# flybirdxx/ComfyUI-SDMatte

Measured on AMD Instinct MI355X. Metric: alpha mattes/sec at 1024x1024, higher is better.
Workload: dtype f16x3

## Files before the change

comfyui-sdmatte_amd/csrc/sdm_engine.cpp:

```cpp
#include "sdm_common.h"
#include "k_conv.h"
#include "k_gemm.h"
#include "k_norm.h"
#include "k_attn.h"
#include "k_misc.h"
#include "k_trimap.h"
#include "k_cclabel.h"
#include "k_foreground.h"
#include "k_guided.h"
#include "k_temporal.h"
#include "k_motion.h"
#include "k_defocus.h"
#include "k_plate.h"
#include "k_harmonize.h"
#include "k_key.h"
#include "k_metrics.h"
#include "k_roi.h"
#include "k_canvas.h"
#include "k_boxes.h"
#include "k_tiles.h"
#include "k_distance.h"
#include "../../include/sdmatte.h"

#include <algorithm>
// ... 65 lines not shown
  {"gemm_p3", 1, 1, "transformer-block Linear layers on the plane-fed GEMM (k_gemm.h): pre-split operand planes from LayerNorm / GroupNorm / attention / GEGLU, LDS-DMA only (the W3 weight copies are built when a model is built)"},
  {"gemm_p3_tile", 0, 0, "row tile of the plane-fed GEMM: 0 by shape, 256 / 128 / 64 forced"},
  {"gemm_p3_attn", 1, 1, "d=64 attention cores write the operand planes of to_out themselves (0: fp32 result + one conversion pass)"},
  {"gemm_p3_persist", 1, 1, "plane-fed GEMM: persistent blocks that prefetch the next tile's first chunk underneath the epilogue (0: one block per tile, n > 1: a grid of n blocks - tests)"},
  {"gemm_p3_ablate", 0, 0, "bench only: 1 no MFMAs, 2 no DMAs behind the prologue, 4 no epilogue (sdm_bench_gemm_p3)"},
  {"conv_up_phase", 1, 1, "up-sampling 3x3 convs (Upsample2D) as four 2x2-tap phase convs on the plane-fed GEMM (k_gemm.h, UP): 0 off (the 3x3 kernels on the up-sampled image), 1 the launches with at least two 256-row tiles per CU (up_phase_wins: measured), 2 every eligible launch (tests).  0 / non-0 is read when a model is built: the phase matrices are a derived weight layout"},
  {"conv_epi", 4, 4, "F8 kernels' epilogue: 4 register-direct stores + residual as accumulator init, 3 residual init only, 0 LDS-staged"},
  {"conv_xtile", 1, 1, "F8 3x3: cross-tile prefetch by the producer waves"},
  {"conv_f8_tpb", 0, 0, "F8: tiles per block (0 = by queue depth)"},
  {"conv_dma", 1, 1, "3x3 stride-1 256x128 tile: weights by LDS-DMA"},
  {"conv_dma_all", 0, 0, "keep a stage-ordered weight copy for every wide 3x3 layer, not only the split-precision ones (read when a model is built)"},
  {"conv_pc", -1, -1, "producer / consumer form of the split-precision DMA kernel: -1 by channel count, 0 off, 1 on"},
  {"conv_pc_min_cin", 256, 256, "conv_pc = -1: smallest Cin that takes the producer / consumer form"},
  {"conv_db", 0, 0, "512x128 double-buffered tile where the queue is deep"},
  {"trimap_skip", 1, 1, "VAE encoder, trimap images: output tiles inside a constant region of the trimap are not multiplied (k_misc.h cmask_*; exact). 0 = every tile"},
  {"conv_band_rows", 0, 0, "tile rows per XCD band of the convs that leave constant tiles out (0 = by image height)"},
  {"trimap_skip_min_rows", 512, 512, "smallest output height at which constant tiles are left out (measured at 1024^2: the 1024- and 512-row levels gain 3.7 + 1.6 ms, the 256-row level loses 0.7: too few of its 32 x 128-pixel tiles lie inside one region)"},
  {"conv_splitk", -1, -1, "split-K of the register-staged conv / GEMM kernels: -1 by shape (few tiles, long K), 0 off, n >= 2 forced where the shape allows"},
  {"force_cfg0", 0, 0, "always the 256x128 tile for 3x3 stride 1 (tests: fused GroupNorm at tiny sizes)"},
  {"no_gn_fuse", 0, 0, "never fuse the GroupNorm apply into the consuming conv"},
  {"split_lds_pad", 0, 0, "extra dynamic LDS of the register-staged split kernels (forces one block per CU)"},
  {"attn_f8", 1, 1, "Q.K^T residual terms of the d=64 split-precision attention on fp8 MFMAs"},
  {"attn_dense", 0, 0, "walk every key tile of the trimap-biased self-attention"},
  {"attn_pv_split", 0, 0, "residual terms of P.V too (fully split attention; tests)"},
  {"attn_nw", 0, 0, "waves per d=64 attention block: 0 by launch size, 4, 8"},
  {"attn_pipe", 1, 1, "8-wave split-precision d=64 attention: two-tile software pipeline"},
  {"attn_pipe4", 1, 1, "the same pipeline for the 4-wave launches (two K / three V^T buffers)"},
  {"attn_pp", 1, 1, "split-precision d=64 attention with fp32 output as a ping-pong of the block's wave halves (attn_d64_pp_kernel, 256 query rows per block): 0 off, 1 on, 2 on without the static priority of the younger half, 3 on with per-segment priority flips"},
  {"attn_pp_min_blocks", 128, 128, "attn_pp: launches with fewer 256-row blocks than this keep the 4-wave pipelines (0 in tests: the ping-pong kernel at any size)"},
  {"attn_ksplit", 0, 0, "key split of the d=64 split-precision attention: 0 by launch size (blocks that do not fill the chip's block slots a whole number of times), 1 off, 2 / 4 forced, 3 forced on the ping-pong kernel (ignored elsewhere: those launches run unsplit)"},
// ... 473 lines not shown
#endif
};

struct sdm_ctx {
  sdm_config cfg;
  int device = 0;
  const unsigned char* dbg_cmask = nullptr;
  void* stream = nullptr;
  bool own_stream = false;
  std::string err;
  std::vector<ConvL> convs;
  std::vector<NormL> norms;
  std::unordered_map<std::string, Slot> slots;
  std::vector<std::string> slot_order;
  unsigned char* warena = nullptr;
  size_t warena_bytes = 0, canon_bytes = 0;
  std::vector<float> hostblob;
  int64_t n_loaded = 0, n_ignored = 0;
  std::vector<std::string> missing;
  bool finalized = false;
  void* stage = nullptr;
  size_t stage_bytes = 0;
  struct LoadSlot {
    void* host = nullptr; void* dev = nullptr; size_t cap = 0; bool busy = false;
#ifndef SDM_EMU
    hipEvent_t done = nullptr;
#endif
  };
  static const int kLoadSlots = 3;
  LoadSlot load_ring[kLoadSlots];
// ... 267 lines not shown
  const int nl = c.unet_layers_per_block + 1;
  for (int i = 0; i < 4; ++i) {
    const int prev_out = output_channel;
    output_channel = uc[3 - i];
    const int input_channel = uc[3 - std::min(i + 1, 3)];
    for (int j = 0; j < nl; ++j) {
      const int res_skip = (j == nl - 1) ? input_channel : output_channel;
      const int resnet_in = (j == 0) ? prev_out : output_channel;
      e->u_up_res[i].push_back(B.resnet("unet.up_blocks." + S(i) + ".resnets." + S(j), resnet_in + res_skip, output_channel, te));
      if (i > 0) e->u_up_tf[i].push_back(B.transformer("unet.up_blocks." + S(i) + ".attentions." + S(j), output_channel, c.unet_heads[3 - i], ctx));
    }
    if (i < 3) e->u_up_us.push_back(B.conv_named("unet.up_blocks." + S(i) + ".upsamplers.0.conv", 9, output_channel, output_channel, true, 0, 0, 1));
  }
  e->u_norm_out = B.norm_named("unet.conv_norm_out", uc[0]);
  e->u_conv_out = B.conv_named("unet.conv_out", 9, uc[0], c.unet_out_channels);
  e->canon_bytes = B.woff;
  e->warena_bytes = B.woff + B.doff;
}

static const size_t kAsideOff = (size_t)1 << 62;

static void arena_diverged(sdm_ctx* e, const char* fmt, size_t i, size_t a, size_t b) {
  if (e->adiverged) return;
  char buf[256];
  snprintf(buf, sizeof(buf), fmt, i, a, b);
  e->adiverged = true; e->adiv_msg = buf;
}

static T talloc_aside(sdm_ctx* e, T t) {
  void* p = nullptr;
// ... 1076 lines not shown
  TRY(conv_simple(e, e->enc_conv_in, xin, &h, e->cfg.vae_channels[0], e->cfg.stream_f32, 1, 0, 0, nullptr, 1.0f, true));
  if (cm) tfree_raw(e, xin.cm_off, xin.cm_bytes);
  for (int i = 0; i < 4; ++i) {
    for (auto& r : e->enc_res[i]) { TRY(resblock(e, r, h, nullptr, eps, &t)); tfree(e, h); h = t; }
    if (i < 3) { TRY(conv_simple(e, e->enc_down[i], h, &t, e->cfg.vae_channels[i], e->cfg.stream_f32, 2, 1, 0, nullptr, 1.0f, true)); tfree(e, h); h = t; }
  }
  TRY(resblock(e, e->enc_mid0, h, nullptr, eps, &t)); tfree(e, h); h = t;
  TRY(vae_attention(e, e->enc_attn, h, &t)); tfree(e, h); h = t;
  TRY(resblock(e, e->enc_mid1, h, nullptr, eps, &t)); tfree(e, h); h = t;
  *moments = talloc(e, h.N, h.H, h.W, 16, e->act_f32);
  { ConvArgs a; a.out = moments; TRY(gn_conv(e, e->norms[e->enc_norm_out], e->convs[e->enc_conv_out], h, nullptr, 1, eps, a)); }
  tfree(e, h);
  return 0;
}

static int vae_decode(sdm_ctx* e, const T& z, T* dec) {
  const float eps = e->cfg.vae_eps;
  T h, t;
  TRY(conv_simple(e, e->dec_conv_in, z, &h, e->cfg.vae_channels[3], e->cfg.stream_f32, 1, 0, 0, nullptr, 1.0f, true));
  TRY(resblock(e, e->dec_mid0, h, nullptr, eps, &t)); tfree(e, h); h = t;
  TRY(vae_attention(e, e->dec_attn, h, &t)); tfree(e, h); h = t;
  TRY(resblock(e, e->dec_mid1, h, nullptr, eps, &t)); tfree(e, h); h = t;
  for (int i = 0; i < 4; ++i) {
    for (auto& r : e->dec_res[i]) { TRY(resblock(e, r, h, nullptr, eps, &t)); tfree(e, h); h = t; }
    if (i < 3) { TRY(conv_simple(e, e->dec_up[i], h, &t, e->cfg.vae_channels[3 - i], e->cfg.stream_f32, 1, 0, 1, nullptr, 1.0f, true)); tfree(e, h); h = t; }
  }
  *dec = talloc(e, h.N, h.H, h.W, 4, 1);
  { ConvArgs a; a.out = dec; TRY(gn_conv(e, e->norms[e->dec_norm_out], e->convs[e->dec_conv_out], h, nullptr, 1, eps, a)); }
  tfree(e, h);
  return 0;
}

static bool level_patch_tokens(sdm_ctx* e, int k, int H, int W, bool option_on) {
  if (!option_on || !sdm_patch_tokens_ok(H, W)) return false;
  const int pf = unet_attn_plane_fmt(e);
  bool ok = true;
  if (k < 3) for (auto& t : e->u_down_tf[k]) ok = ok && transformer_p3(e, t, pf);
  if (k == 3) ok = ok && transformer_p3(e, e->u_midtf, pf);
  if (k < 3) for (auto& t : e->u_up_tf[3 - k]) ok = ok && transformer_p3(e, t, pf);
  return ok;
}

static int unet_forward(sdm_ctx* e, const T& uin, bool masked, float* const* bias_lvl, int* const* tiles_lvl, const bool* patch_lvl, T* out) {
// ... 73 lines not shown
  T uin = talloc(e, B, lh, lw, 16, e->act_f32);
  if (!e->dry) SDM_CHECK_DEV(e, dev_memset(uin.p, 0, uin.bytes, e->stream));
  for (int half = 0; half < 2; ++half) {
    T mv = moments; mv.N = B;
    if (!e->dry) mv.p = (unsigned char*)moments.p + (size_t)half * B * lh * lw * 16 * fmt_bytes(moments.f32);
    ConvArgs a; a.in0 = &mv; a.out = &uin; a.out_ch_off = half * 4; a.cout_valid = 4; a.out_scale = c.vae_scaling_factor;
    TRY(op_conv(e, e->convs[e->quant], a));
  }
  tfree(e, moments);
  T lat;
  TRY(unet_forward(e, uin, use_mask, bias_lvl, tiles_lvl, patch_lvl, &lat));
  tfree(e, uin);
  for (int k = 3; k >= 0; --k) { tfree(e, tilebuf[k]); tfree(e, biasbuf[k]); }
  T z;
  TRY(conv_simple(e, e->post_quant, lat, &z, 16, e->act_f32)); tfree(e, lat);
  T dec;
  TRY(vae_decode(e, z, &dec)); tfree(e, z);
  *alpha = talloc(e, B, SH, SW, 1, 1);
  if (!e->dry)
    SDM_LAUNCH(alpha_out_kernel, dim3((unsigned)(((long)B * SH * SW + 255) / 256)), dim3(256), 0, e->stream, (const float*)dec.p, (float*)alpha->p,
               (long)B * SH * SW);
  tfree(e, dec);
  return 0;
}

static int trimap_check(sdm_ctx* e, int B, int H, int W, int erode_px, int dilate_px) {
  if (B <= 0 || H <= 0 || W <= 0) SDM_FAIL(e, SDM_ERR_INVALID, "trimap from mask: bad mask size %dx%dx%d", B, H, W);
  if (erode_px < 0 || erode_px > SDM_TRIMAP_MAX_RADIUS || dilate_px < 0 || dilate_px > SDM_TRIMAP_MAX_RADIUS)
    SDM_FAIL(e, SDM_ERR_INVALID, "trimap from mask: erode_px = %d, dilate_px = %d outside 0 .. %d", erode_px, dilate_px, SDM_TRIMAP_MAX_RADIUS);
  if ((double)B * H * sdm_cdiv(W, SDM_TRIMAP_ROWS_W) >= 2147483647.0) SDM_FAIL(e, SDM_ERR_INVALID, "trimap from mask: %dx%dx%d is too large", B, H, W);
  return 0;
}

static int trimap_cols_rows(int B, int H, int W, int R) {
  int rows = 128;
  while (rows > 32 && ((long)B * sdm_cdiv(H, rows) * sdm_cdiv(W, SDM_TRIMAP_COLS_W) < 512 || trimap_cols_smem(rows, R) > 48 * 1024)) rows /= 2;
  return rows;
// ... 333 lines not shown
  (void)hipEventCreate(&e->ev0); (void)hipEventCreate(&e->ev1);
  (void)hipEventCreateWithFlags(&e->ev_in, hipEventDisableTiming); (void)hipEventCreateWithFlags(&e->ev_out, hipEventDisableTiming);
#endif
  void* p = nullptr;
  if (dev_malloc(&p, e->warena_bytes) != 0) { g_create_err = "cannot allocate weight arena"; sdm_destroy(e); return SDM_ERR_NOMEM; }
  e->warena = (unsigned char*)p;
  dev_memset(e->warena, 0, e->warena_bytes, e->stream);
  for (auto& L : e->convs) {
    L.w = (half_t*)(e->warena + L.w_off); L.b = (float*)(e->warena + L.b_off);
    if (L.split) L.w_lo = (half_t*)(e->warena + L.wlo_off);
    if (L.wdma_bytes) L.w_dma = (half_t*)(e->warena + e->canon_bytes + L.wdma_off);
    if (L.w3_bytes) L.w3 = e->warena + e->canon_bytes + L.w3_off;
    if (L.wup_bytes) L.wup = e->warena + e->canon_bytes + L.wup_off;
  }
  for (auto& n : e->norms) { n.g = (float*)(e->warena + n.g_off); n.b = (float*)(e->warena + n.b_off); }
  for (auto& t : e->tembs) {
    void* q = nullptr;
    if (dev_malloc(&q, (size_t)kMinVariantRows * t.cout_pad * 4) != 0) { g_create_err = "cannot allocate temb tables"; sdm_destroy(e); return SDM_ERR_NOMEM; }
    t.table = (float*)q;
    dev_memset(q, 0, (size_t)kMinVariantRows * t.cout_pad * 4, e->stream);
  }
  e->variant_cap = kMinVariantRows;
  dev_sync(e->stream);
  *out = e;
  return SDM_OK;
}

void sdm_destroy(sdm_ctx* e) {
  if (e) dev_use(e->device);
  if (!e) return;
// ... 267 lines not shown
                 (const half_t*)L->w, (const half_t*)L->w_lo, L->wup, L->Cin_pad, L->Cout_pad, ldexpf(1.0f, -L->w_exp), ldexpf(1.0f, L->up_exp));
    if (!L->w_dma) continue;
    const size_t total = (size_t)L->Cin_pad * L->ntaps * L->Cout_pad;
    if (L->f8)
      SDM_LAUNCH(derive_conv_weight_f8_kernel, dim3((unsigned)std::min<size_t>((total / 4 + 255) / 256, 65535)), dim3(256), 0, e->stream,
                 (const half_t*)L->w, (const half_t*)L->w_lo, (unsigned char*)L->w_dma, L->Cin_pad, L->Cout_pad, L->ntaps, ldexpf(1.0f, -L->w_exp),
                 ldexpf(1.0f, L->f8_exp));
    else
      SDM_LAUNCH(derive_conv_weight_dma_kernel, dim3((unsigned)std::min<size_t>((total * (L->split ? 2 : 1) + 255) / 256, 65535)), dim3(256), 0, e->stream,
                 (const half_t*)L->w, (const half_t*)L->w_lo, L->w_dma, L->Cin_pad, L->Cout_pad, L->split ? 2 : 1);
  }
  SDM_CHECK_DEV(e, dev_sync(e->stream));
  return 0;
}

static void load_ring_release(sdm_ctx* e) {
#ifndef SDM_EMU
  for (auto& sl : e->load_ring) {
    if (sl.busy) { (void)hipEventSynchronize(sl.done); sl.busy = false; }
    if (sl.host) (void)hipHostFree(sl.host);
    if (sl.dev) dev_free(sl.dev);
    if (sl.done) (void)hipEventDestroy(sl.done);
    sl.host = sl.dev = nullptr; sl.cap = 0; sl.done = nullptr;
  }
#else
  (void)e;
#endif
}

int sdm_finalize_weights(sdm_ctx* e) {
  if (e) dev_use(e->device);
  if (!e) return SDM_ERR_INVALID;
  SDM_CHECK_DEV(e, dev_sync(e->stream));
  load_ring_release(e);
  { int rc = fold_cross_kv(e); if (rc) return rc; }
  {
    std::vector<ConvL*> all;
    for (auto& L : e->convs) all.push_back(&L);
    int rc = derive_layers(e, all);
    if (rc) return rc;
  }
  e->missing.clear();
  for (auto& k : e->slot_order) if (!e->slots[k].loaded) e->missing.push_back(k);
  e->variants.clear();
  e->finalized = true;
  return SDM_OK;
}

int sdm_weight_stats(sdm_ctx* e, int64_t* n_loaded, int64_t* n_missing, int64_t* n_ignored) {
  if (!e) return SDM_ERR_INVALID;
  if (n_loaded) *n_loaded = e->n_loaded;
  if (n_missing) *n_missing = (int64_t)e->missing.size();
  if (n_ignored) *n_ignored = e->n_ignored;
  return SDM_OK;
// ... 1335 lines not shown
```

comfyui-sdmatte_amd/csrc/sdm_hooks.h:

```cpp
#pragma once

struct DevBuf {
  void* p = nullptr;
  DevBuf() = default;
  DevBuf(DevBuf&& o) noexcept : p(o.p) { o.p = nullptr; }
  ~DevBuf() { if (p) dev_free(p); }
  int alloc(size_t n) { return dev_malloc(&p, n); }
  int alloc0(size_t n, void* stream) { const int rc = alloc(n); return rc ? rc : dev_memset(p, 0, n, stream); }
};

struct RestoreInt { int& s; int v; ~RestoreInt() { s = v; } };

struct TempLayer {
  enum { kDma = 1, kW3 = 2, kUp = 4 };
  sdm_ctx* e;
  ConvL L;
  DevBuf w, w_lo, b, w_dma, w3, wup;
  explicit TempLayer(sdm_ctx* c) : e(c) {}
  ~TempLayer() { dev_sync(e->stream); }
  int init(const char* name, int ntaps, int I, int O, int geglu, int split, int layouts, const float* wsrc, const float* bias) {
    L = make_layer(name, ntaps, I, O, geglu, split);
    layer_choose_layouts(L, layouts & kDma, layouts & kDma, layouts & kW3, layouts & kUp);
    SDM_CHECK_DEV(e, w.alloc0(L.w_bytes(), e->stream));
    SDM_CHECK_DEV(e, b.alloc0(L.b_bytes(), e->stream));
// ... 236 lines not shown
  TRY(tl.init("op_up", 9, C, O, 0, 1, TempLayer::kDma | TempLayer::kUp, w, bias));
  return run_two_pass(e, [&]() -> int {
    T tin = view(x, N, H, W, C, 1), to = view(out, N, 2 * H, 2 * W, O, 1);
    to.want_stats = true;
    ConvArgs a; a.in0 = &tin; a.out = &to; a.up = 1;
    TRY(op_conv(e, tl.L, a));
    if (!e->dry) {
      SDM_CHECK_DEV(e, dev_memcpy_d2d(stats, to.stats, (size_t)N * to.srows * O * 2 * 4, e->stream));
      *srows = to.srows;
    }
    if (to.sbytes) { tfree_raw(e, to.soff, to.sbytes); to.sbytes = 0; }
    return 0;
  });
}

int sdm_debug_set_input_cmask(sdm_ctx* e, const unsigned char* mask) {
  if (!e) return SDM_ERR_INVALID;
  e->dbg_cmask = mask;
  return SDM_OK;
}

int sdm_op_conv(sdm_ctx* e, const void* in0, const void* in1, int C0, int C1, int in_f32, int N, int Hin, int Win, int up, int stride,
                int pad_mode, int ntaps, const float* w, const float* bias, int O, void* out, int out_f32, const void* res, int res_f32,
                int geglu, float out_scale, int tile_cfg) {
  return sdm_op_conv_ex(e, in0, in1, C0, C1, in_f32, N, Hin, Win, up, stride, pad_mode, ntaps, w, bias, O, out, out_f32, res, res_f32, geglu,
                        out_scale, tile_cfg, 0, nullptr, nullptr, 0.0f, 32, 0);
}


int sdm_debug_run_layer(sdm_ctx* e, const char* layer_name, const float* x, int N, int H, int W, float* out, int Cout) {
// ... 477 lines not shown
```

comfyui-sdmatte_amd/engine.py:

```python
import ctypes as C
import os

import numpy as np
import torch

from .config import SDMatteConfig

_HERE = os.path.dirname(os.path.abspath(__file__))
LIB_PATH = os.path.join(_HERE, "csrc", "libsdmatte_hip.so")

SDM_PTR_HOST, SDM_PTR_DEVICE = 0, 1
SDM_F32, SDM_F16, SDM_BF16 = 0, 1, 2
_DT = {torch.float32: SDM_F32, torch.float16: SDM_F16, torch.bfloat16: SDM_BF16}


class SdmConfig(C.Structure):
    _fields_ = [
        ("vae_channels", C.c_int32 * 4), ("vae_layers_per_block", C.c_int32),
        ("unet_channels", C.c_int32 * 4), ("unet_heads", C.c_int32 * 4), ("unet_layers_per_block", C.c_int32),
        ("cross_attention_dim", C.c_int32), ("unet_in_channels", C.c_int32), ("unet_out_channels", C.c_int32),
        ("bbox_embeddings_input_dim", C.c_int32), ("groups", C.c_int32),
        ("vae_eps", C.c_float), ("unet_res_eps", C.c_float), ("unet_tf_gn_eps", C.c_float), ("unet_ln_eps", C.c_float),
        ("vae_scaling_factor", C.c_float), ("attn_mask_value", C.c_float),
        ("stream_f32", C.c_int32), ("point_embeddings_input_dim", C.c_int32), ("precise_mask", C.c_int32), ("reserved", C.c_int32 * 5),
# ... 36 lines not shown
    c.unet_tf_gn_eps, c.unet_ln_eps = cfg.unet_tf_gn_eps, cfg.unet_ln_eps
    c.vae_scaling_factor, c.attn_mask_value = cfg.vae_scaling_factor, cfg.attn_mask_value
    c.stream_f32 = 1 if stream_f32 else 0
    c.point_embeddings_input_dim = cfg.point_embeddings_input_dim
    c.precise_mask = precise_mask_of(precision)
    return c


EXPORTS = [
    "sdm_default_config", "sdm_create", "sdm_destroy", "sdm_last_error", "sdm_load_tensor", "sdm_finalize_weights",
    "sdm_weight_stats", "sdm_missing_key", "sdm_weight_blob_bytes", "sdm_export_weight_blob", "sdm_import_weight_blob",
    "sdm_host_blob_bytes", "sdm_export_host_blob", "sdm_import_host_blob", "sdm_forward", "sdm_forward_ex", "sdm_forward_rect", "sdm_apply_matte", "sdm_apply_matte_node",
    "sdm_make_trimap", "sdm_clean_mask", "sdm_apply_matte_mask", "sdm_subject_roi", "sdm_apply_matte_roi", "sdm_subject_boxes", "sdm_apply_matte_boxes", "sdm_band_tiles", "sdm_apply_matte_tiles", "sdm_estimate_foreground", "sdm_refine_alpha_guided", "sdm_compose_canvas",
    "sdm_distance_field", "sdm_offset_mask", "sdm_outline", "sdm_smooth_alpha_temporal", "sdm_smooth_alpha_motion", "sdm_defocus_background", "sdm_fill_background", "sdm_harmonize", "sdm_screen_colour", "sdm_chroma_key", "sdm_matte_metrics",
    "sdm_synchronize", "sdm_release_memory", "sdm_resident_bytes", "sdm_weight_bytes", "sdm_last_forward_ms", "sdm_profile_enable", "sdm_profile_count", "sdm_profile_get", "sdm_profile_dump",
    "sdm_op_conv", "sdm_op_conv_ex", "sdm_op_conv_stats", "sdm_op_gn_partials", "sdm_op_gn_tables", "sdm_op_conv_up_stats", "sdm_op_gemm_p3", "sdm_debug_run_layer", "sdm_debug_set_input_cmask", "sdm_debug_temb_row", "sdm_conv_num_cfgs", "sdm_bench_conv", "sdm_bench_attn", "sdm_bench_gemm_p3", "sdm_op_groupnorm", "sdm_op_layernorm", "sdm_op_attention", "sdm_op_attention_ex", "sdm_op_attention_split", "sdm_op_attention_split_ex", "sdm_debug_attn_plan", "sdm_op_resize_aa",
    "sdm_op_mask_bias", "sdm_debug_patch_token_map", "sdm_op_groupnorm_p3", "sdm_op_gemm_p3_tokens", "sdm_op_mask_bias_tokens", "sdm_op_active_tiles",
    "sdm_op_cross_patch_planes", "sdm_op_cross_patch_planes_ex", "sdm_op_attention_shared", "sdm_debug_cross_attention", "sdm_op_cross_core",
    "sdm_set_option", "sdm_get_option", "sdm_reset_options", "sdm_option_name", "sdm_option_help", "sdm_kernel_counts", "sdm_kernel_counts_reset",
]


class Bindings:

    def __init__(self, cdll):
        self.dll = cdll
        vp, i32, i64, f32 = C.c_void_p, C.c_int, C.c_int64, C.c_float
        sig = {
            "sdm_default_config": (None, [C.POINTER(SdmConfig)]),
            "sdm_create": (i32, [C.POINTER(vp), i32, C.POINTER(SdmConfig)]),
            "sdm_destroy": (None, [vp]),
# ... 44 lines not shown
            "sdm_profile_enable": (i32, [vp, i32]),
            "sdm_profile_count": (i32, [vp]),
            "sdm_profile_dump": (C.c_char_p, [vp]),
            "sdm_profile_get": (i32, [vp, i32, C.POINTER(C.c_char_p), C.POINTER(f32), C.POINTER(i64), C.POINTER(C.c_double),
                                      C.POINTER(C.c_double)]),
            "sdm_op_conv": (i32, [vp, vp, vp, i32, i32, i32, i32, i32, i32, i32, i32, i32, i32, vp, vp, i32, vp, i32, vp, i32, i32,
                                  f32, i32]),
            "sdm_op_conv_ex": (i32, [vp, vp, vp, i32, i32, i32, i32, i32, i32, i32, i32, i32, i32, vp, vp, i32, vp, i32, vp, i32, i32,
                                     f32, i32, i32, vp, vp, f32, i32, i32]),
            "sdm_op_conv_stats": (i32, [vp, vp, vp, i32, i32, i32, i32, i32, i32, i32, i32, i32, i32, vp, vp, i32, vp, i32, vp, i32, i32,
                                        f32, i32, i32, vp, vp, f32, i32, i32, vp, i32, vp, i32, vp, i32, C.POINTER(i32)]),
            "sdm_op_gn_partials": (i32, [vp, vp, i32, vp, i32, i32, i32, i32, i32, i32, vp, vp, f32, vp, vp]),
            "sdm_op_gn_tables": (i32, [vp, vp, vp, i32, i32, i32, i32, i32, i32, vp, vp, f32, vp, vp]),
            "sdm_op_gemm_p3": (i32, [vp, vp, i32, i32, i32, i32, vp, vp, i32, i32, vp, vp, vp, f32, i32, vp, vp, C.POINTER(i32)]),
            "sdm_op_conv_up_stats": (i32, [vp, vp, i32, i32, i32, i32, vp, vp, i32, vp, vp, C.POINTER(i32)]),
            "sdm_debug_run_layer": (i32, [vp, C.c_char_p, vp, i32, i32, i32, vp, i32]),
            "sdm_debug_set_input_cmask": (i32, [vp, vp]),
            "sdm_debug_temb_row": (i32, [vp, i32, i32, vp, vp, i32]),
            "sdm_conv_num_cfgs": (i32, [i32, i32]),
            "sdm_bench_conv": (f32, [vp] + [i32] * 11),
            "sdm_bench_attn": (f32, [vp] + [i32] * 7),
            "sdm_bench_gemm_p3": (f32, [vp, C.c_long, i32, i32, i32, i32]),
            "sdm_op_groupnorm": (i32, [vp, vp, vp, i32, i32, i32, i32, i32, i32, vp, vp, f32, i32, vp]),
            "sdm_op_layernorm": (i32, [vp, vp, i32, C.c_long, i32, vp, vp, f32, vp]),
            "sdm_op_attention": (i32, [vp, vp, i32, vp, i32, vp, i32, vp, i32, i32, i32, i32, i32, vp, i32]),
            "sdm_op_attention_ex": (i32, [vp, vp, i32, vp, i32, vp, i32, i32, i32, i32, i32, i32, i32, vp, i32]),
            "sdm_op_attention_split": (i32, [vp, vp, vp, vp, vp, i32, i32, i32, i32, vp]),
            "sdm_op_attention_split_ex": (i32, [vp, vp, vp, vp, vp, vp, i32, i32, i32, i32, i32, vp, vp]),
            "sdm_debug_attn_plan": (i32, [i32] * 10 + [C.c_char_p, i32, C.POINTER(i32)]),
            "sdm_op_resize_aa": (i32, [vp, vp, i32, i32, i32, vp, i32, i32]),
# ... 1200 lines not shown
        return scale, shift

    def op_conv_up_stats(self, x, w, bias=None):
        N, H, W_, Cin = x.shape
        O = w.shape[0]
        x = x.float().contiguous(); w = w.float().contiguous()
        b = bias.float().contiguous() if bias is not None else None
        out = torch.empty(N, 2 * H, 2 * W_, O, dtype=torch.float32, device=x.device)
        srows_max = 8 * (((H + 2) * (W_ + 2) + 63) // 64) + 4 * ((H + 1) // 2) * ((W_ + 3) // 4)
        stats = torch.zeros(N * srows_max * O * 2, dtype=torch.float32, device=x.device)
        srows = C.c_int(0)
        self._check(self.lib.sdm_op_conv_up_stats(self.h, _ptr(x), N, H, W_, Cin, _ptr(w), _ptr(b), O, _ptr(out), _ptr(stats), C.byref(srows)),
                    "sdm_op_conv_up_stats")
        return out, stats[:N * srows.value * O * 2].view(N, srows.value, O, 2)

    def op_gemm_p3(self, x, w, bias=None, mode=0, res=None, ln=None, lo_cols=-1):
        N, H, W_, K = x.shape
        O = w.shape[0]
        x = x.float().contiguous(); w = w.float().contiguous()
        b = bias.float().contiguous() if bias is not None else None
        r = res.float().contiguous() if res is not None else None
        gam = ln[0].float().contiguous() if ln is not None else None
        bet = ln[1].float().contiguous() if ln is not None else None
        Cst = O // 2 if mode == 1 else O
        if mode == 2:
            out = torch.zeros(2 * N * H * W_ * O, dtype=torch.float16, device=x.device)
        else:
            out = torch.empty(N, H, W_, Cst, dtype=torch.float32, device=x.device)
        srows_max = 2 * ((H * W_ + 63) // 64)
        stats = torch.zeros(N * srows_max * O * 2, dtype=torch.float32, device=x.device) if mode == 4 else None
# ... 176 lines not shown
```

include/sdmatte.h:

```cpp
#ifndef SDMATTE_H_
#define SDMATTE_H_

#include <stddef.h>
#include <stdint.h>

#ifdef __cplusplus
extern "C" {
#endif

typedef struct sdm_ctx sdm_ctx;

enum sdm_status {
  SDM_OK = 0,
  SDM_ERR_INVALID = -1,
  SDM_ERR_HIP = -2,
  SDM_ERR_STATE = -3,
  SDM_ERR_NOMEM = -4,
  SDM_ERR_NODEVICE = -5,
  SDM_ERR_ARENA = -6
};

enum sdm_ptr_kind { SDM_PTR_HOST = 0, SDM_PTR_DEVICE = 1 };
enum sdm_dtype { SDM_F32 = 0, SDM_F16 = 1, SDM_BF16 = 2 };

// ... 231 lines not shown
                   const float* gn_beta, float gn_eps, int gn_groups, int gn_silu);
int sdm_op_conv_stats(sdm_ctx* ctx, const void* in0, const void* in1, int C0, int C1, int in_f32, int N, int Hin, int Win, int up,
                      int stride, int pad_mode, int ntaps, const float* w, const float* bias, int O, void* out, int out_f32,
                      const void* res, int res_f32, int geglu, float out_scale, int tile_cfg, int split, const float* gn_gamma,
                      const float* gn_beta, float gn_eps, int gn_groups, int gn_silu, const float* in_st0, int in_rows0, const float* in_st1,
                      int in_rows1, float* stats, int stats_cap, int* srows);
int sdm_op_gn_partials(sdm_ctx* ctx, const float* st0, int rows0, const float* st1, int rows1, int C0, int C1, int N, int HW, int groups,
                       const float* gamma, const float* beta, float eps, float* scale, float* shift);
int sdm_op_gn_tables(sdm_ctx* ctx, const void* x0, const void* x1, int C0, int C1, int in_f32, int N, int HW, int groups, const float* gamma,
                     const float* beta, float eps, float* scale, float* shift);
float sdm_bench_gemm_p3(sdm_ctx* ctx, long M, int K, int O, int epi_flags, int iters);
int sdm_op_gemm_p3(sdm_ctx* ctx, const float* x, int N, int H, int W, int K, const float* w, const float* bias, int O, int mode, const float* res,
                   const float* ln_gamma, const float* ln_beta, float ln_eps, int lo_cols, void* out, float* stats, int* srows);
int sdm_op_conv_up_stats(sdm_ctx* ctx, const float* x, int N, int H, int W, int C, const float* w, const float* bias, int O, float* out, float* stats,
                         int* srows);
int sdm_debug_set_input_cmask(sdm_ctx* ctx, const unsigned char* mask);
int sdm_debug_run_layer(sdm_ctx* ctx, const char* layer_name, const float* x_nhwc, int N, int H, int W, float* out_nhwc, int Cout);
int sdm_debug_temb_row(sdm_ctx* ctx, int temb_index, int is_trans, const float* coords4, float* out_host, int cout);
float sdm_bench_attn(sdm_ctx* ctx, int B, int heads, int Lq, int Lk, int qt, int ablate, int iters);
float sdm_bench_conv(sdm_ctx* ctx, int N, int H, int W, int Cin, int Cout, int ntaps, int stride, int in_f32, int tile_cfg, int ablate, int iters);
int sdm_op_groupnorm(sdm_ctx* ctx, const void* in0, const void* in1, int C0, int C1, int in_f32, int N, int HW, int groups,
                     const float* gamma, const float* beta, float eps, int silu, void* out_f16);
int sdm_op_layernorm(sdm_ctx* ctx, const void* x, int in_f32, long rows, int C, const float* gamma, const float* beta,
                     float eps, void* out_f16);
int sdm_op_attention(sdm_ctx* ctx, const void* q, int ldq, const void* k, int ldk, const void* v, int ldv, const float* bias,
                     int B, int heads, int Lq, int Lk, int D, void* out, int ldo);
int sdm_op_attention_ex(sdm_ctx* ctx, const void* q, int ldq, const void* k, int ldk, const void* v, int ldv, int B, int heads, int Lq, int Lk, int D, int out_f32,
                        void* out, int ldo);
int sdm_op_attention_split(sdm_ctx* ctx, const float* q, const float* k, const float* v, const float* bias, int B, int heads, int Lq, int Lk, float* out);
int sdm_op_attention_split_ex(sdm_ctx* ctx, const float* q, const float* k, const float* v, const float* bias, const int* tiles, int B, int heads, int Lq,
// ... 23 lines not shown
```

Before: 22.00.

## Fuse VAE decoder tail into one alpha kernel on mean-folded conv_out weights

New measurement: 22.05 (median of 6 runs). About the same (+0.2%).

```diff
diff --git a/comfyui-sdmatte_amd/csrc/k_vae_ends.h b/comfyui-sdmatte_amd/csrc/k_vae_ends.h
--- /dev/null
+++ b/comfyui-sdmatte_amd/csrc/k_vae_ends.h
@@ -0,0 +1,138 @@
+#pragma once
+#include "sdm_common.h"
+
+#define SDM_DA_TH 30
+#define SDM_DA_TW 32
+#define SDM_DA_RH (SDM_DA_TH + 2)
+#define SDM_DA_RW (SDM_DA_TW + 2)
+#define SDM_DA_RWP (SDM_DA_RW + 1)
+#define SDM_DA_U 4
+
+struct DecAlphaParams {
+  const float* x;
+  const float* scale;
+  const float* shift;
+  const float* wt;
+  float* alpha;
+  int N, H, W;
+};
+
+template <int LPP>
+SDM_DEV_INLINE float dec_alpha_group_sum(float v) {
+#ifdef SDM_EMU
+#pragma unroll
+  for (int m = 1; m < LPP; m <<= 1) v += __shfl_xor(v, m);
+#else
+  v = SDM_DPP_ADD(v, 0xB1);
+  v = SDM_DPP_ADD(v, 0x4E);
+  if (LPP >= 8) v = SDM_DPP_ADD(v, 0x141);
+  if (LPP >= 16) v = SDM_DPP_ADD(v, 0x140);
+#endif
+  return v;
+}
+
+SDM_DEV_INLINE float dec_alpha_silu(float x) {
+  const float d = 1.0f + sdm_exp2(fminf(-x * SDM_LOG2E, 126.0f));
+  float r = sdm_rcp(d);
+  r = fmaf(fmaf(-d, r, 1.0f), r, r);
+  return x * r;
+}
+
+template <int C>
+__global__ void __launch_bounds__(256, 2) dec_alpha_kernel(DecAlphaParams p) {
+  constexpr int LPP = C / 8, PPB = 256 / LPP, NPIX = SDM_DA_RH * SDM_DA_RW, STEPS = (NPIX + PPB - 1) / PPB, NB = (STEPS + SDM_DA_U - 1) / SDM_DA_U;
+  static_assert(C == 32 || C == 64 || C == 128, "dec_alpha_kernel: 4, 8 or 16 lanes per pixel");
+  SDM_SHARED float t[9 * SDM_DA_RH * SDM_DA_RWP];
+  const int tid = threadIdx.x, j = tid % LPP, g = tid / LPP;
+  const int n = blockIdx.z, y0 = blockIdx.y * SDM_DA_TH, x0 = blockIdx.x * SDM_DA_TW;
+  const int H = p.H, W = p.W;
+  const int th = min(SDM_DA_TH, H - y0), tw = min(SDM_DA_TW, W - x0);
+  f32x4 w[9][2], sc[2], sh[2];
+#pragma unroll
+  for (int h = 0; h < 2; ++h) {
+#pragma unroll
+    for (int tap = 0; tap < 9; ++tap) w[tap][h] = *(const f32x4*)(p.wt + tap * C + 4 * (j + h * LPP));
+    sc[h] = *(const f32x4*)(p.scale + (size_t)n * C + 4 * (j + h * LPP));
+    sh[h] = *(const f32x4*)(p.shift + (size_t)n * C + 4 * (j + h * LPP));
+  }
+  const float* img = p.x + (size_t)n * H * W * C;
+  auto place = [&](int pix, int& pr, int& pc) -> bool {
+    pr = pix / SDM_DA_RW; pc = pix - pr * SDM_DA_RW;
+    const int gy = y0 - 1 + pr, gx = x0 - 1 + pc;
+    return pix < NPIX && pr < th + 2 && pc < tw + 2 && gy >= 0 && gy < H && gx >= 0 && gx < W;
+  };
+  auto load = [&](f32x4 (&a)[SDM_DA_U][2], int batch) {
+#pragma unroll
+    for (int u = 0; u < SDM_DA_U; ++u) {
+      int pr, pc;
+      (void)place((batch * SDM_DA_U + u) * PPB + g, pr, pc);
+      pr = min(pr, SDM_DA_RH - 1);
+      const int gy = min(max(y0 - 1 + pr, 0), H - 1), gx = min(max(x0 - 1 + pc, 0), W - 1);
+      const f32x4* s = (const f32x4*)(img + ((size_t)gy * W + gx) * C) + j;
+      a[u][0] = s[0]; a[u][1] = s[LPP];
+    }
+  };
+  auto compute = [&](const f32x4 (&a)[SDM_DA_U][2], int batch) {
+#pragma unroll
+    for (int u = 0; u < SDM_DA_U; ++u) {
+      const int pix = (batch * SDM_DA_U + u) * PPB + g;
+      int pr, pc;
+      const bool ok = place(pix, pr, pc);
+      float v[8];
+#pragma unroll
+      for (int h = 0; h < 2; ++h)
+#pragma unroll
+        for (int k = 0; k < 4; ++k) v[h * 4 + k] = dec_alpha_silu(fmaf(a[u][h][k], sc[h][k], sh[h][k]));
+      float r[9];
+#pragma unroll
+      for (int tap = 0; tap < 9; ++tap) {
+        float s = v[0] * w[tap][0][0];
+#pragma unroll
+        for (int k = 1; k < 8; ++k) s = fmaf(v[k], w[tap][k >> 2][k & 3], s);
+        r[tap] = dec_alpha_group_sum<LPP>(s);
+      }
+      float* dst = t + pr * SDM_DA_RWP + pc;
+      if (LPP >= 9) {
+        float sel = r[0];
+#pragma unroll
+        for (int tap = 1; tap < 9; ++tap) sel = (j == tap) ? r[tap] : sel;
+        if (pix < NPIX && j < 9) dst[j * (SDM_DA_RH * SDM_DA_RWP)] = ok ? sel : 0.0f;
+      } else {
+#pragma unroll
+        for (int tap = 0; tap < 9; ++tap)
+          if (pix < NPIX && (tap % LPP) == j) dst[tap * (SDM_DA_RH * SDM_DA_RWP)] = ok ? r[tap] : 0.0f;
+      }
+    }
+  };
+  f32x4 a0[SDM_DA_U][2], a1[SDM_DA_U][2];
+  load(a0, 0);
+  for (int b = 0; b < NB; b += 2) {
+    load(a1, b + 1);
+    compute(a0, b);
+    load(a0, b + 2);
+    if (b + 1 < NB) compute(a1, b + 1);
+  }
+  __syncthreads();
+  const float bias = p.wt[9 * C];
+  const int oy = tid >> 3, ox = (tid & 7) * 4;
+  if (oy < th && ox < tw) {
+    double acc[4] = {0.0, 0.0, 0.0, 0.0};
+#pragma unroll
+    for (int tap = 0; tap < 9; ++tap) {
+      const float* src = t + tap * (SDM_DA_RH * SDM_DA_RWP) + (oy + tap / 3) * SDM_DA_RWP + ox + tap % 3;
+#pragma unroll
+      for (int k = 0; k < 4; ++k) acc[k] += (double)src[k];
+    }
+    float o[4];
+#pragma unroll
+    for (int k = 0; k < 4; ++k) o[k] = (SDM_MED3((float)(acc[k] + (double)bias), -1.0f, 1.0f) + 1.0f) * 0.5f;
+    float* dst = p.alpha + ((size_t)n * H + (y0 + oy)) * W + x0 + ox;
+    if ((W & 3) == 0) {
+      const f32x4 o4 = {o[0], o[1], o[2], o[3]};
+      *(f32x4*)dst = o4;
+    } else {
+#pragma unroll
+      for (int k = 0; k < 4; ++k) if (ox + k < tw) dst[k] = o[k];
+    }
+  }
+}
diff --git a/comfyui-sdmatte_amd/csrc/sdm_engine.cpp b/comfyui-sdmatte_amd/csrc/sdm_engine.cpp
--- a/comfyui-sdmatte_amd/csrc/sdm_engine.cpp
+++ b/comfyui-sdmatte_amd/csrc/sdm_engine.cpp
@@ -4,6 +4,7 @@
 #include "k_norm.h"
 #include "k_attn.h"
 #include "k_misc.h"
+#include "k_vae_ends.h"
 #include "k_trimap.h"
 #include "k_cclabel.h"
 #include "k_foreground.h"
@@ -103,6 +104,7 @@
   {"conv_pc_min_cin", 256, 256, "conv_pc = -1: smallest Cin that takes the producer / consumer form"},
   {"conv_db", 0, 0, "512x128 double-buffered tile where the queue is deep"},
   {"trimap_skip", 1, 1, "VAE encoder, trimap images: output tiles inside a constant region of the trimap are not multiplied (k_misc.h cmask_*; exact). 0 = every tile"},
+  {"vae_ends", 1, 1, "VAE decoder, callers that want the alpha: conv_norm_out + SiLU + conv_out + the mean / clamp of the three decoded channels as ONE streaming launch on the mean weights (k_vae_ends.h dec_alpha_kernel; fp32 activations, 32 / 64 / 128 channels).  0 = the 3-channel conv_out on the thin conv kernel + alpha_out_kernel.  Read per forward (the mean-weight table is derived whenever weights are finalised: 4.6 KB)"},
   {"conv_band_rows", 0, 0, "tile rows per XCD band of the convs that leave constant tiles out (0 = by image height)"},
   {"trimap_skip_min_rows", 512, 512, "smallest output height at which constant tiles are left out (measured at 1024^2: the 1024- and 512-row levels gain 3.7 + 1.6 ms, the 256-row level loses 0.7: too few of its 32 x 128-pixel tiles lie inside one region)"},
   {"conv_splitk", -1, -1, "split-K of the register-staged conv / GEMM kernels: -1 by shape (few tiles, long K), 0 off, n >= 2 forced where the shape allows"},
@@ -606,6 +608,8 @@
   std::unordered_map<std::string, Slot> slots;
   std::vector<std::string> slot_order;
   unsigned char* warena = nullptr;
+  size_t dec_alpha_off = 0;
+  float* dec_alpha_w = nullptr;
   size_t warena_bytes = 0, canon_bytes = 0;
   std::vector<float> hostblob;
   int64_t n_loaded = 0, n_ignored = 0;
@@ -903,6 +907,7 @@
   }
   e->u_norm_out = B.norm_named("unet.conv_norm_out", uc[0]);
   e->u_conv_out = B.conv_named("unet.conv_out", 9, uc[0], c.unet_out_channels);
+  e->dec_alpha_off = B.doff; B.doff += rupz(((size_t)9 * vc[0] + 1) * 4, 256);
   e->canon_bytes = B.woff;
   e->warena_bytes = B.woff + B.doff;
 }
@@ -2009,7 +2014,51 @@
   return 0;
 }
 
-static int vae_decode(sdm_ctx* e, const T& z, T* dec) {
+static bool dec_alpha_ok(const T& h) { return opt("vae_ends") != 0 && h.f32 == 1 && (h.C == 32 || h.C == 64 || h.C == 128); }
+
+static int decode_alpha(sdm_ctx* e, const NormL& n, const ConvL& L, const float* wt, const T& h, float eps, T* alpha) {
+  if (h.C != n.C || h.C != L.Cin_pad) SDM_FAIL(e, SDM_ERR_INVALID, "decode_alpha: C %d != %d / %d", h.C, n.C, L.Cin_pad);
+  const long npix = h.rows();
+  if (!dec_alpha_ok(h)) {
+    T dec = talloc(e, h.N, h.H, h.W, 4, 1);
+    { ConvArgs a; a.out = &dec; TRY(gn_conv(e, n, L, h, nullptr, 1, eps, a)); }
+    *alpha = talloc(e, h.N, h.H, h.W, 1, 1);
+    if (!e->dry) {
+      prof_begin(e, "alpha_out", 0, (double)npix * 20);
+      count_kernel("alpha_out");
+      SDM_LAUNCH(alpha_out_kernel, dim3((unsigned)((npix + 255) / 256)), dim3(256), 0, e->stream, (const float*)dec.p, (float*)alpha->p, npix);
+      prof_end(e);
+    }
+    tfree(e, dec);
+    return 0;
+  }
+  if (h.N > 65535 || sdm_cdiv(h.H, SDM_DA_TH) > 65535) SDM_FAIL(e, SDM_ERR_INVALID, "decode_alpha: %d images of %d rows exceed the launch grid", h.N, h.H);
+  *alpha = talloc(e, h.N, h.H, h.W, 1, 1);
+  T scratch; float* scale; float* shift;
+  TRY(gn_scale_shift(e, h.p, nullptr, h.C, 0, h.f32, h.N, h.H * h.W, e->cfg.groups, n.g, n.b, eps, h.stats, h.srows, nullptr, 0, h.sbytes != 0, &scratch, &scale,
+                     &shift));
+  if (!e->dry) {
+    DecAlphaParams p;
+    p.x = (const float*)h.p; p.scale = scale; p.shift = shift; p.wt = wt; p.alpha = (float*)alpha->p; p.N = h.N; p.H = h.H; p.W = h.W;
+    const dim3 grid((unsigned)sdm_cdiv(h.W, SDM_DA_TW), (unsigned)sdm_cdiv(h.H, SDM_DA_TH), (unsigned)h.N);
+    char d[160];
+    d[0] = 0;
+    if (e->prof_on) snprintf(d, sizeof(d), "%s N=%d H=%d W=%d Cin=%d -> alpha", L.name.c_str(), h.N, h.H, h.W, h.C);
+    prof_begin(e, "dec_alpha", 2.0 * (double)npix * h.C * 9, (double)npix * h.C * 4 + (double)npix * 4, d);
+    count_kernel("dec_alpha");
+    if (h.C == 128) SDM_LAUNCH(dec_alpha_kernel<128>, grid, dim3(256), 0, e->stream, p);
+    else if (h.C == 64) SDM_LAUNCH(dec_alpha_kernel<64>, grid, dim3(256), 0, e->stream, p);
+    else SDM_LAUNCH(dec_alpha_kernel<32>, grid, dim3(256), 0, e->stream, p);
+#ifndef SDM_EMU
+    { const hipError_t le = hipGetLastError(); if (le != hipSuccess) SDM_FAIL(e, SDM_ERR_HIP, "dec_alpha: launch failed: %s", hipGetErrorString(le)); }
+#endif
+    prof_end(e);
+  }
+  tfree(e, scratch);
+  return 0;
+}
+
+static int vae_decode(sdm_ctx* e, const T& z, T* alpha) {
   const float eps = e->cfg.vae_eps;
   T h, t;
   TRY(conv_simple(e, e->dec_conv_in, z, &h, e->cfg.vae_channels[3], e->cfg.stream_f32, 1, 0, 0, nullptr, 1.0f, true));
@@ -2020,8 +2069,7 @@
     for (auto& r : e->dec_res[i]) { TRY(resblock(e, r, h, nullptr, eps, &t)); tfree(e, h); h = t; }
     if (i < 3) { TRY(conv_simple(e, e->dec_up[i], h, &t, e->cfg.vae_channels[3 - i], e->cfg.stream_f32, 1, 0, 1, nullptr, 1.0f, true)); tfree(e, h); h = t; }
   }
-  *dec = talloc(e, h.N, h.H, h.W, 4, 1);
-  { ConvArgs a; a.out = dec; TRY(gn_conv(e, e->norms[e->dec_norm_out], e->convs[e->dec_conv_out], h, nullptr, 1, eps, a)); }
+  TRY(decode_alpha(e, e->norms[e->dec_norm_out], e->convs[e->dec_conv_out], e->dec_alpha_w, h, eps, alpha));
   tfree(e, h);
   return 0;
 }
@@ -2125,13 +2173,7 @@
   for (int k = 3; k >= 0; --k) { tfree(e, tilebuf[k]); tfree(e, biasbuf[k]); }
   T z;
   TRY(conv_simple(e, e->post_quant, lat, &z, 16, e->act_f32)); tfree(e, lat);
-  T dec;
-  TRY(vae_decode(e, z, &dec)); tfree(e, z);
-  *alpha = talloc(e, B, SH, SW, 1, 1);
-  if (!e->dry)
-    SDM_LAUNCH(alpha_out_kernel, dim3((unsigned)(((long)B * SH * SW + 255) / 256)), dim3(256), 0, e->stream, (const float*)dec.p, (float*)alpha->p,
-               (long)B * SH * SW);
-  tfree(e, dec);
+  TRY(vae_decode(e, z, alpha)); tfree(e, z);
   return 0;
 }
 
@@ -2495,6 +2537,7 @@
     if (L.wup_bytes) L.wup = e->warena + e->canon_bytes + L.wup_off;
   }
   for (auto& n : e->norms) { n.g = (float*)(e->warena + n.g_off); n.b = (float*)(e->warena + n.b_off); }
+  e->dec_alpha_w = (float*)(e->warena + e->canon_bytes + e->dec_alpha_off);
   for (auto& t : e->tembs) {
     void* q = nullptr;
     if (dev_malloc(&q, (size_t)kMinVariantRows * t.cout_pad * 4) != 0) { g_create_err = "cannot allocate temb tables"; sdm_destroy(e); return SDM_ERR_NOMEM; }
@@ -2792,6 +2835,34 @@
   return 0;
 }
 
+static int derive_dec_alpha(sdm_ctx* e, const ConvL& L, float* dst) {
+  if (L.ntaps != 9 || L.O < 1) SDM_FAIL(e, SDM_ERR_INVALID, "%s: mean weights are for a 3x3 layer", L.name.c_str());
+  const size_t n = L.w_bytes() / 2;
+  std::vector<half_t> hi(n), lo;
+  std::vector<float> b((size_t)L.Cout_pad);
+  SDM_CHECK_DEV(e, dev_memcpy_d2h(hi.data(), L.w, n * 2, e->stream));
+  if (L.w_lo) { lo.resize(n); SDM_CHECK_DEV(e, dev_memcpy_d2h(lo.data(), L.w_lo, n * 2, e->stream)); }
+  SDM_CHECK_DEV(e, dev_memcpy_d2h(b.data(), L.b, b.size() * 4, e->stream));
+  SDM_CHECK_DEV(e, dev_sync(e->stream));
+  std::vector<float> tab((size_t)9 * L.Cin_pad + 1);
+  const double unit = std::ldexp(1.0, -L.w_exp) / (double)L.O;
+  for (int tap = 0; tap < 9; ++tap)
+    for (int ci = 0; ci < L.Cin_pad; ++ci) {
+      double acc = 0.0;
+      for (int co = 0; co < L.O; ++co) {
+        const size_t idx = (((size_t)(ci / 16) * 9 + tap) * L.Cout_pad + co) * 16 + ci % 16;
+        acc += (double)(float)hi[idx] + (L.w_lo ? (double)(float)lo[idx] : 0.0);
+      }
+      tab[(size_t)tap * L.Cin_pad + ci] = (float)(acc * unit);
+    }
+  double bs = 0.0;
+  for (int co = 0; co < L.O; ++co) bs += (double)b[(size_t)co];
+  tab[(size_t)9 * L.Cin_pad] = (float)(bs / (double)L.O);
+  SDM_CHECK_DEV(e, dev_memcpy_h2d(dst, tab.data(), tab.size() * 4, e->stream));
+  SDM_CHECK_DEV(e, dev_sync(e->stream));
+  return 0;
+}
+
 static void load_ring_release(sdm_ctx* e) {
 #ifndef SDM_EMU
   for (auto& sl : e->load_ring) {
@@ -2816,6 +2887,8 @@
     std::vector<ConvL*> all;
     for (auto& L : e->convs) all.push_back(&L);
     int rc = derive_layers(e, all);
+    if (rc) return rc;
+    rc = derive_dec_alpha(e, e->convs[e->dec_conv_out], e->dec_alpha_w);
     if (rc) return rc;
   }
   e->missing.clear();
diff --git a/comfyui-sdmatte_amd/csrc/sdm_hooks.h b/comfyui-sdmatte_amd/csrc/sdm_hooks.h
--- a/comfyui-sdmatte_amd/csrc/sdm_hooks.h
+++ b/comfyui-sdmatte_amd/csrc/sdm_hooks.h
@@ -274,6 +274,28 @@
   });
 }
 
+int sdm_op_dec_alpha(sdm_ctx* e, const float* x, int N, int H, int W, int C, const float* w, const float* bias, int O, const float* gn_gamma, const float* gn_beta,
+                     float gn_eps, float* alpha) {
+  if (e) dev_use(e->device);
+  if (!e || !x || !w || !gn_gamma || !gn_beta || !alpha || N < 1 || H < 1 || W < 1 || O < 1) return SDM_ERR_INVALID;
+  if (C % 16) SDM_FAIL(e, SDM_ERR_INVALID, "sdm_op_dec_alpha: C %% 16 required");
+  DevBuf wt;
+  TempLayer tl(e);
+  TRY(tl.init("op_dec_alpha", 9, C, O, 0, 1, 0, w, bias));
+  SDM_CHECK_DEV(e, wt.alloc(((size_t)9 * C + 1) * 4));
+  TRY(derive_dec_alpha(e, tl.L, (float*)wt.p));
+  NormL nl; nl.C = C; nl.g = const_cast<float*>(gn_gamma); nl.b = const_cast<float*>(gn_beta);
+  RestoreInt keep_act{e->act_f32, e->act_f32};
+  e->act_f32 = 1;
+  return run_two_pass(e, [&]() -> int {
+    T tx = view(x, N, H, W, C, 1), ta;
+    TRY(decode_alpha(e, nl, tl.L, (const float*)wt.p, tx, gn_eps, &ta));
+    if (!e->dry) SDM_CHECK_DEV(e, dev_memcpy_d2d(alpha, ta.p, (size_t)N * H * W * 4, e->stream));
+    tfree(e, ta);
+    return 0;
+  });
+}
+
 int sdm_debug_set_input_cmask(sdm_ctx* e, const unsigned char* mask) {
   if (!e) return SDM_ERR_INVALID;
   e->dbg_cmask = mask;
diff --git a/comfyui-sdmatte_amd/engine.py b/comfyui-sdmatte_amd/engine.py
--- a/comfyui-sdmatte_amd/engine.py
+++ b/comfyui-sdmatte_amd/engine.py
@@ -74,7 +74,7 @@
     "sdm_make_trimap", "sdm_clean_mask", "sdm_apply_matte_mask", "sdm_subject_roi", "sdm_apply_matte_roi", "sdm_subject_boxes", "sdm_apply_matte_boxes", "sdm_band_tiles", "sdm_apply_matte_tiles", "sdm_estimate_foreground", "sdm_refine_alpha_guided", "sdm_compose_canvas",
     "sdm_distance_field", "sdm_offset_mask", "sdm_outline", "sdm_smooth_alpha_temporal", "sdm_smooth_alpha_motion", "sdm_defocus_background", "sdm_fill_background", "sdm_harmonize", "sdm_screen_colour", "sdm_chroma_key", "sdm_matte_metrics",
     "sdm_synchronize", "sdm_release_memory", "sdm_resident_bytes", "sdm_weight_bytes", "sdm_last_forward_ms", "sdm_profile_enable", "sdm_profile_count", "sdm_profile_get", "sdm_profile_dump",
-    "sdm_op_conv", "sdm_op_conv_ex", "sdm_op_conv_stats", "sdm_op_gn_partials", "sdm_op_gn_tables", "sdm_op_conv_up_stats", "sdm_op_gemm_p3", "sdm_debug_run_layer", "sdm_debug_set_input_cmask", "sdm_debug_temb_row", "sdm_conv_num_cfgs", "sdm_bench_conv", "sdm_bench_attn", "sdm_bench_gemm_p3", "sdm_op_groupnorm", "sdm_op_layernorm", "sdm_op_attention", "sdm_op_attention_ex", "sdm_op_attention_split", "sdm_op_attention_split_ex", "sdm_debug_attn_plan", "sdm_op_resize_aa",
+    "sdm_op_conv", "sdm_op_conv_ex", "sdm_op_conv_stats", "sdm_op_gn_partials", "sdm_op_gn_tables", "sdm_op_conv_up_stats", "sdm_op_dec_alpha", "sdm_op_gemm_p3", "sdm_debug_run_layer", "sdm_debug_set_input_cmask", "sdm_debug_temb_row", "sdm_conv_num_cfgs", "sdm_bench_conv", "sdm_bench_attn", "sdm_bench_gemm_p3", "sdm_op_groupnorm", "sdm_op_layernorm", "sdm_op_attention", "sdm_op_attention_ex", "sdm_op_attention_split", "sdm_op_attention_split_ex", "sdm_debug_attn_plan", "sdm_op_resize_aa",
     "sdm_op_mask_bias", "sdm_debug_patch_token_map", "sdm_op_groupnorm_p3", "sdm_op_gemm_p3_tokens", "sdm_op_mask_bias_tokens", "sdm_op_active_tiles",
     "sdm_op_cross_patch_planes", "sdm_op_cross_patch_planes_ex", "sdm_op_attention_shared", "sdm_debug_cross_attention", "sdm_op_cross_core",
     "sdm_set_option", "sdm_get_option", "sdm_reset_options", "sdm_option_name", "sdm_option_help", "sdm_kernel_counts", "sdm_kernel_counts_reset",
@@ -149,6 +149,7 @@
             "sdm_op_gn_tables": (i32, [vp, vp, vp, i32, i32, i32, i32, i32, i32, vp, vp, f32, vp, vp]),
             "sdm_op_gemm_p3": (i32, [vp, vp, i32, i32, i32, i32, vp, vp, i32, i32, vp, vp, vp, f32, i32, vp, vp, C.POINTER(i32)]),
             "sdm_op_conv_up_stats": (i32, [vp, vp, i32, i32, i32, i32, vp, vp, i32, vp, vp, C.POINTER(i32)]),
+            "sdm_op_dec_alpha": (i32, [vp, vp, i32, i32, i32, i32, vp, vp, i32, vp, vp, f32, vp]),
             "sdm_debug_run_layer": (i32, [vp, C.c_char_p, vp, i32, i32, i32, vp, i32]),
             "sdm_debug_set_input_cmask": (i32, [vp, vp]),
             "sdm_debug_temb_row": (i32, [vp, i32, i32, vp, vp, i32]),
@@ -1379,6 +1380,17 @@
                     "sdm_op_conv_up_stats")
         return out, stats[:N * srows.value * O * 2].view(N, srows.value, O, 2)
 
+    def op_dec_alpha(self, x, w, bias, gamma, beta, eps):
+        N, H, W_, Cin = x.shape
+        O = w.shape[0]
+        x = x.float().contiguous(); w = w.float().contiguous()
+        b = bias.float().contiguous() if bias is not None else None
+        gamma = gamma.float().contiguous(); beta = beta.float().contiguous()
+        alpha = torch.empty(N, H, W_, dtype=torch.float32, device=x.device)
+        self._check(self.lib.sdm_op_dec_alpha(self.h, _ptr(x), N, H, W_, Cin, _ptr(w), _ptr(b), O, _ptr(gamma), _ptr(beta), float(eps), _ptr(alpha)),
+                    "sdm_op_dec_alpha")
+        return alpha
+
     def op_gemm_p3(self, x, w, bias=None, mode=0, res=None, ln=None, lo_cols=-1):
         N, H, W_, K = x.shape
         O = w.shape[0]
diff --git a/include/sdmatte.h b/include/sdmatte.h
--- a/include/sdmatte.h
+++ b/include/sdmatte.h
@@ -269,6 +269,8 @@
                    const float* ln_gamma, const float* ln_beta, float ln_eps, int lo_cols, void* out, float* stats, int* srows);
 int sdm_op_conv_up_stats(sdm_ctx* ctx, const float* x, int N, int H, int W, int C, const float* w, const float* bias, int O, float* out, float* stats,
                          int* srows);
+int sdm_op_dec_alpha(sdm_ctx* ctx, const float* x, int N, int H, int W, int C, const float* w, const float* bias, int O, const float* gn_gamma,
+                     const float* gn_beta, float gn_eps, float* alpha);
 int sdm_debug_set_input_cmask(sdm_ctx* ctx, const unsigned char* mask);
 int sdm_debug_run_layer(sdm_ctx* ctx, const char* layer_name, const float* x_nhwc, int N, int H, int W, float* out_nhwc, int Cout);
 int sdm_debug_temb_row(sdm_ctx* ctx, int temb_index, int is_trans, const float* coords4, float* out_host, int cout);
```
